# nncarlson/nka

Hardware: AMD Instinct MI355X
Metric: NKA updates/sec + achieved HBM GB/s at n=1e8, m=20 fp64; 1/2/4/8 GPUs (higher is better)
Workload: dtype f64

## Files before the change

### nka_amd/csrc/handles.hpp

```cpp
#pragma once

#include "../../include/nka_hip.h"
#include "../../include/nka_hip_ext.h"
#include "../../include/nka_hip_vec.h"
#include "nka_kernels.hpp"
#include "host_logic.hpp"
#include "rccl_dl.hpp"

#include <hip/hip_runtime.h>

#include <cstdint>
#include <string>
#include <vector>

namespace nka_detail {
int set_error(int code, const std::string &msg);
std::string last_error();
bool &span_check_failed();
int check_device_span(const void *p, int64_t n, const char *what);
void invalidate_span_cache();
void register_allocation(const void *p, size_t bytes, const void *owner);
void unregister_owner(const void *owner);
void unregister_allocation(const void *p);

// ... 41 lines not shown
  bool swap_pending = false;
  int64_t swap_seq = 0;
  const double *last_acc = nullptr;
  std::vector<void *> extra_allocs;
  nka_host::BufferBook book;
  bool captured = false;
  bool solve63_raised = false;
  bool poisoned = false;
  int num_cu = 256;
  int bpc[2] = {0, 0};
  char devname[64] = {0};
  int pa_pipe = -1;
  int pb_pipe = -1;
  int pb_flags = 0;
  int pb_tile = -1;
  int pb_tickets = -1;
  double *chain_pred = nullptr;
  void *chain_summ = nullptr;
  long long chain_cap = 0;
  int chain_many = -1;
  int chain_walk = 0;
  int fail_after_solve = 0;
  int prime_pad = -1;
  bool state_in_global = false;
  bool serial_solve = false;
  int sum_order = NKA_HIP_SUMS_AUTO;
  bool debug = false;
  nka_hip_allreduce_fn allreduce = nullptr;
  void *allreduce_ctx = nullptr;
  ncclComm_t comm = nullptr;
  nka::P2P p2p{};
  void *p2p_mail = nullptr;
  std::vector<void *> p2p_opened;
  void *p2p_dev = nullptr;
  int p2p_ranks = 0;
  bool p2p_fused = false;
  int pa_normed = 0;
  int shard_rank = -1, shard_n = 0;
  bool needs_comm = false;
  nka_hip_host_dot_fn host_dot = nullptr;
  void *host_dot_ctx = nullptr;
  int timing_cap = 0;
  int64_t timing_count = 0;
  int timing_stride = 1;
  int64_t update_seq = 0;
  bool timing_this = false;
// ... 21 lines not shown
```

### nka_amd/csrc/lab.hip

```cpp
#include "handles.hpp"
#include "../../include/nka_hip_diag.h"

#include <algorithm>
#include <string>

using namespace nka;
using namespace nka_detail;

extern "C" {

int nka_hip_get_stamps(nka_hip_t a, double *out16) {
  if (!a || !out16) return fail(NKA_HIP_EINVAL, "null argument");
  HIP_TRY(hipSetDevice(a->device));
  HIP_TRY(hipMemcpyAsync(out16, a->ctl.stamps(), sizeof(double) * kStamps, hipMemcpyDeviceToHost, a->stream));
  HIP_TRY(hipStreamSynchronize(a->stream));
  return 0;
}

int nka_hip_set_grid(nka_hip_t a, int32_t pa, int32_t pb) {
  if (!a) return fail(NKA_HIP_EINVAL, "null handle");
  const int32_t v[2] = {pa, pb};
  for (int i = 0; i < 2; i++) {
    if (v[i] < 0 || v[i] * a->num_cu > kMaxGrid) return fail(NKA_HIP_EINVAL, "blocks per CU out of range");
    a->bpc[i] = v[i];
// ... 73 lines not shown
  } else if (k == "pa_pipe") {
    if (value != -1 && value != 0 && !(value > 200 && value <= 204))
      return fail(NKA_HIP_EINVAL, "pa_pipe: -1 (auto), 0 (every load of a tile in flight), 201..204 (rolling window, 1..4 blocks per CU)");
    a->pa_pipe = value;
  } else if (k == "pb_tile") {
    if (value != -1 && value != 1 && value != 2) return fail(NKA_HIP_EINVAL, "pb_tile: -1 (auto), 1, 2");
    a->pb_tile = value;
  } else if (k == "pb_tickets") {
    if (value != -1 && value != 0 && value != 1 && value != 2 && value != 4 && value != 8)
      return fail(NKA_HIP_EINVAL, "pb_tickets: -1 (auto), 0 (static tile mapping), 1, 2, 4, 8 (ticket counters)");
    a->pb_tickets = value;
  } else if (k == "fail_after_solve") {
    a->fail_after_solve = value != 0;
  } else if (k == "prime_pad") {
    if (value < -1 || value > 1) return fail(NKA_HIP_EINVAL, "prime_pad: -1, 0, 1");
    a->prime_pad = value;
  } else if (k == "chain_many") {
    if (value < -1 || value > 1) return fail(NKA_HIP_EINVAL, "chain_many: -1, 0, 1");
    a->chain_many = value;
  } else if (k == "chain_walk") {
    a->chain_walk = value != 0;
  } else if (k == "serial_solve") {
    a->serial_solve = value != 0;
  } else if (k == "list_word") {
    a->word_off = value == 0;
  } else {
    return fail(NKA_HIP_EINVAL, "unknown tuning key: " + k);
  }
  return 0;
}

int nka_hip_vec_set_tuning(nka_hip_vec_ws_t ws, const char *key, int32_t value) {
  if (!ws || !key) return fail(NKA_HIP_EINVAL, "null argument");
  if (std::string(key) == "tickets") {
    if (value != -1 && value != 0 && value != 1 && value != 2 && value != 4 && value != 8)
      return fail(NKA_HIP_EINVAL, "tickets: -1 (auto), 0 (static tile mapping), 1, 2, 4, 8 (ticket counters)");
    ws->ticket_groups = value;
    return 0;
  }
  return fail(NKA_HIP_EINVAL, std::string("unknown tuning key: ") + key);
}

}
```

### nka_amd/csrc/nka_hip.hip

```cpp
#include "handles.hpp"

#include <dlfcn.h>

#include <algorithm>
#include <atomic>
#include <chrono>
#include <cmath>
#include <cstdio>
#include <cstdlib>
#include <cstring>
#include <map>
#include <mutex>
#include <set>
#include <string>
#include <vector>

using namespace nka;

namespace {
thread_local std::string g_err;
}

namespace nka_detail {
int set_error(int code, const std::string &msg) {
// ... 314 lines not shown
constexpr int kTimingEvents = 4;

int list_bound_now(nka_hip_state *a) {
  if (a->word_off || !a->list_word) return a->list_ub;
  const unsigned long long w = __atomic_load_n(a->list_word, __ATOMIC_ACQUIRE);
  return nka_host::list_bound_from_word(a->list_ub, w, a->seq, a->word_valid_after, a->relaxed_after);
}

constexpr size_t kMaxDynamicLds = 160 * 1024;
constexpr int kMaxMvec = 140;
static_assert(lst_smem_bytes(kMaxMvec) <= kMaxDynamicLds && lst_smem_bytes(kMaxMvec + 1) > kMaxDynamicLds,
              "kMaxMvec out of step with lst_smem_bytes");

int record(nka_hip_state *a, int i) {
  if (i == 0) a->timing_this = a->timing_cap > 0 && (a->update_seq++ % a->timing_stride) == 0;
  if (!a->timing_this) return 0;
  const int slot = (int)(a->timing_count % a->timing_cap);
  HIP_TRY(hipEventRecord(a->ev[(size_t)slot * kTimingEvents + i], a->stream));
  return 0;
}

}

extern "C" {

const char *nka_hip_last_error(void) { return g_err.c_str(); }

void nka_hip_invalidate_pointer_cache(void) { nka_detail::invalidate_span_cache(); }

int nka_hip_create(nka_hip_t *out, int64_t vlen_local, int32_t mvec, double vtol, int32_t flavor,
                   int32_t device, void *stream) {
  if (!out) return fail(NKA_HIP_EINVAL, "nka_hip_create: out is NULL");
  *out = nullptr;
  if (mvec <= 0) return fail(NKA_HIP_EINVAL, "nka_hip_create: mvec must be > 0");
  if (vlen_local < 0) return fail(NKA_HIP_EINVAL, "nka_hip_create: vlen must be >= 0");
  if (!(vtol > 0.0)) return fail(NKA_HIP_EINVAL, "nka_hip_create: vtol must be > 0");
  if (flavor == NKA_HIP_FLAVOR_DEFAULT) {
    flavor = NKA_HIP_FLAVOR_C;
    if (const char *e = getenv("NKA_HIP_FLAVOR")) {
      const std::string v(e);
      if (v == "f08" || v == "F08" || v == "0") flavor = NKA_HIP_FLAVOR_F08;
      else if (v == "f08vec" || v == "F08VEC" || v == "f08_vector" || v == "1") flavor = NKA_HIP_FLAVOR_F08_VECTOR;
      else if (v == "c" || v == "C" || v == "compact" || v == "2") flavor = NKA_HIP_FLAVOR_C;
      else if (!v.empty()) return fail(NKA_HIP_EINVAL, "NKA_HIP_FLAVOR: expected f08, f08vec or c, got '" + v + "'");
    }
  }
// ... 191 lines not shown

static int fetch_tables(nka_hip_t a, std::vector<long long> &pc, Ctl &t) {
  pc.assign((size_t)a->ctl.pc_count(), 0);
  HIP_TRY(hipMemcpyAsync(pc.data(), a->ctl.pc, sizeof(long long) * pc.size(), hipMemcpyDeviceToHost, a->stream));
  HIP_TRY(hipStreamSynchronize(a->stream));
  t = a->ctl;
  t.pc = pc.data();
  return 0;
}
static const double *slot_buffer(nka_hip_t a, const Ctl *tables, bool v, int slot) {
  if (tables) return buffer_at(a, v ? tables->vtab()[slot] : tables->wtab()[slot]);
  return (v ? a->vs.v : a->vs.w) + (size_t)(slot - 1) * a->vs.stride;
}
static __global__ void k_plan_pointers_from_slots(Ctl ctl) {
  if (threadIdx.x != 0 || blockIdx.x != 0) return;
  const int n = ctl.ic[IC_PLAN_NOLDER];
  for (int j = 0; j < n; j++) ctl.plan_w()[j] = ctl.wtab()[ctl.plan_slots()[j]];
  ctl.pc[PC_FIRST_W] = ctl.wtab()[ctl.ic[IC_PLAN_FIRST]];
}

int nka_hip_clone(nka_hip_t src, nka_hip_t *out) {
  if (!src || !out) return fail(NKA_HIP_EINVAL, "nka_hip_clone: null argument");
  *out = nullptr;
  nka_hip_t b = nullptr;
  if (int rc = nka_hip_create(&b, src->n, src->mvec, src->vtol, src->flavor, src->device, (void *)src->stream)) return rc;
  if (b->vs.stride != src->vs.stride || b->ctl.ic_count() != src->ctl.ic_count() || b->ctl.dc_count() != src->ctl.dc_count()) {
    nka_hip_destroy(b);
    return fail(NKA_HIP_ESTATE, "nka_hip_clone: storage geometry differs");
  }
  const size_t slot_bytes = (size_t)src->vs.stride * sizeof(double) * (size_t)(src->mvec + 1);
  hipStream_t s = src->stream;
  hipError_t e = hipSuccess;
  if (!src->swapped) {
    e = hipMemcpyAsync(b->vs.v, src->vs.v, slot_bytes, hipMemcpyDeviceToDevice, s);
    if (e == hipSuccess) e = hipMemcpyAsync(b->vs.w, src->vs.w, slot_bytes, hipMemcpyDeviceToDevice, s);
  } else {
    std::vector<long long> pc;
    Ctl t{};
    if (int rc = fetch_tables(src, pc, t)) {
      nka_hip_destroy(b);
      return rc;
    }
    const size_t nb = sizeof(double) * (size_t)src->n;
    for (int k = 1; k <= src->mvec + 1 && e == hipSuccess && nb > 0; k++) {
      e = hipMemcpyAsync(b->vs.w + (size_t)(k - 1) * b->vs.stride, buffer_at(src, t.wtab()[k]), nb, hipMemcpyDeviceToDevice, s);
      if (e == hipSuccess)
        e = hipMemcpyAsync(b->vs.v + (size_t)(k - 1) * b->vs.stride, buffer_at(src, t.vtab()[k]), nb, hipMemcpyDeviceToDevice, s);
    }
  }
  if (e == hipSuccess) e = hipMemcpyAsync(b->ctl.ic, src->ctl.ic, sizeof(int32_t) * src->ctl.ic_count(), hipMemcpyDeviceToDevice, s);
  if (e == hipSuccess) e = hipMemcpyAsync(b->ctl.dc, src->ctl.dc, sizeof(double) * src->ctl.dc_count(), hipMemcpyDeviceToDevice, s);
  if (e == hipSuccess) {
    hipLaunchKernelGGL(k_plan_pointers_from_slots, dim3(1), dim3(1), 0, s, b->ctl);
    e = hipGetLastError();
  }
  if (e != hipSuccess) {
    nka_hip_destroy(b);
    return fail(NKA_HIP_EHIP, std::string("nka_hip_clone: ") + hipGetErrorString(e));
  }
  b->pending = src->pending;
  b->list_ub = src->list_ub;
  b->bpc[0] = src->bpc[0];
  b->bpc[1] = src->bpc[1];
  b->pa_pipe = src->pa_pipe;
  b->pb_pipe = src->pb_pipe;
  b->pb_tile = src->pb_tile;
  b->pb_tickets = src->pb_tickets;
  b->prime_pad = src->prime_pad;
  b->chain_walk = src->chain_walk;
  b->chain_many = src->chain_many;
  b->chain_pred = nullptr; b->chain_summ = nullptr; b->chain_cap = 0;
  b->serial_solve = src->serial_solve;
  b->sum_order = src->sum_order;
  b->shard_rank = src->shard_rank;
  b->shard_n = src->shard_n;
  b->debug = src->debug;
  if (src->allreduce != rccl_allreduce && src->allreduce != p2p_allreduce) {
    b->allreduce = src->allreduce;
    b->allreduce_ctx = src->allreduce_ctx;
    b->needs_comm = src->needs_comm;
  } else {
    b->needs_comm = true;
  }
  b->host_dot = src->host_dot;
  b->host_dot_ctx = src->host_dot_ctx;
  *out = b;
  return 0;
}

int nka_hip_restart(nka_hip_t a) {
  if (!a) return fail(NKA_HIP_EINVAL, "null handle");
  if (a->poisoned) return fail(NKA_HIP_ESTATE, "restart: an earlier update failed after its scalar step had been enqueued: destroy the handle");
  HIP_TRY(hipSetDevice(a->device));
  hipLaunchKernelGGL(k_restart, dim3(1), dim3(kSolveThreads), a->state_in_global ? 0 : lst_smem_bytes(a->mvec), a->stream,
                     a->ctl, a->state_in_global ? 1 : 0);
  HIP_TRY(hipGetLastError());
  a->pending = false;
  a->list_ub = 0;
  a->word_valid_after = a->seq;
  a->relaxed_after.clear();
  return 0;
}

int nka_hip_relax(nka_hip_t a) {
  if (!a) return fail(NKA_HIP_EINVAL, "null handle");
  if (a->poisoned) return fail(NKA_HIP_ESTATE, "relax: an earlier update failed after its scalar step had been enqueued: destroy the handle");
  HIP_TRY(hipSetDevice(a->device));
  hipLaunchKernelGGL(k_relax, dim3(1), dim3(kSolveThreads), a->state_in_global ? 0 : lst_smem_bytes(a->mvec), a->stream,
                     a->ctl, a->state_in_global ? 1 : 0);
  HIP_TRY(hipGetLastError());
  if (a->pending) {
    a->pending = false;
    a->list_ub = std::max(a->list_ub - 1, 0);
    if (!a->word_off && a->list_word) a->relaxed_after.push_back(a->seq);
    if (a->relaxed_after.size() > 4096) a->relaxed_after.erase(a->relaxed_after.begin(), a->relaxed_after.begin() + 2048);
  }
  return 0;
}

int nka_hip_set_vec_tol(nka_hip_t a, double vtol) {
  if (!a) return fail(NKA_HIP_EINVAL, "null handle");
  if (!(vtol > 0.0)) return fail(NKA_HIP_EINVAL, "set_vec_tol: vtol must be > 0");
  HIP_TRY(hipSetDevice(a->device));
  a->vtol = vtol;
  HIP_TRY(hipMemcpyAsync(a->ctl.dc + DC_VTOL, &a->vtol, sizeof(double), hipMemcpyHostToDevice, a->stream));
  HIP_TRY(hipStreamSynchronize(a->stream));
  return 0;
}

static int enqueue_solve(nka_hip_t a, int mode, long long swap_w = kNoBuffer, long long swap_v = kNoBuffer, bool gather = false) {
  hipStream_t s = a->stream;
  const P2P x = gather ? a->p2p : P2P{};
  if (a->mvec + 1 <= kSolveWaveMax && !a->serial_solve) {
    const size_t sm = solve_wave_smem_bytes(a->mvec);
    const int nl = a->mvec + 1;
    const long long id_stride = (a->swapped || a->captured) ? 0 : (long long)a->vs.stride, id_vbase = buffer_offset(a, a->vs.v);
#define ROWS(NL) \
  hipLaunchKernelGGL((k_solve_rows<NL>), dim3(1), dim3(kSolveThreads), sm, s, a->ctl, mode, swap_w, swap_v, id_stride, id_vbase, x)
    if (nl <= 6) ROWS(6);
    else if (nl <= 11) ROWS(11);
    else if (nl <= 21) ROWS(21);
    else if (nl <= 33) ROWS(33);
    else if (nl <= 48) ROWS(48);
    else {
      if (!a->solve63_raised) {
        const hipError_t raised = hipFuncSetAttribute(reinterpret_cast<const void *>(k_solve_rows<63>),
                                                      hipFuncAttributeMaxDynamicSharedMemorySize,
                                                      (int)solve_wave_smem_bytes(kSolveWaveMax - 1));
        if (raised != hipSuccess) return fail(NKA_HIP_EHIP, std::string("raising the dynamic LDS limit failed: ") + hipGetErrorString(raised));
        a->solve63_raised = true;
      }
      ROWS(63);
    }
#undef ROWS
  } else {
    hipLaunchKernelGGL(k_solve, dim3(1), dim3(kSolveThreads), a->state_in_global ? 0 : lst_smem_bytes(a->mvec), s, a->ctl, mode,
                       a->state_in_global ? 1 : 0, 0, swap_w, swap_v, x);
  }
  HIP_TRY(hipGetLastError());
  return 0;
}

}

void nka_detail::enqueue_pa(nka_hip_t a, const double *f, int vec, int older_ub) {
  const int maxl = (vec == 1) ? 4 : (older_ub > kMaxPerPass ? kMaxPerPass : round_up4(older_ub));
  const int npass = std::max(1, (older_ub + maxl - 1) / maxl);
  int pa_pipe = a->pa_pipe;
  const bool exact = vec == 2 && older_ub >= 1 && older_ub <= kMaxPerPass;
  if (pa_pipe < 0) pa_pipe = exact ? 201 : 0;
  if (vec == 2 && npass == 1 && pa_pipe > 200 && pa_pipe < 210) {
    int w = exact ? older_ub : maxl;
    if (a->prime_pad != 0 && heavy_prime(w)) w++;
    launch_dots_win(w, a, f, std::max(1, pa_pipe - 200));
  } else if (vec == 2 && older_ub > kMaxPerPass && a->pa_pipe != 0) {
    const int np = balanced_passes(older_ub);
    std::vector<int> wd((size_t)np);
    balanced_widths(older_ub, np, wd.data());
    for (int p = 0, base = 0; p < np; p++) {
      launch_dots_win(wd[(size_t)p], a, f, a->pa_pipe > 200 ? a->pa_pipe - 200 : 1, base, p, older_ub);
      base += wd[(size_t)p];
    }
  } else {
    for (int p = 0; p < npass; p++) {
      if (vec == 2) launch_dots_w(maxl, a, f, p, npass);
      else launch_dots_1<4, 1>(a, f, p, npass);
    }
  }
// ... 347 lines not shown
  return r;
}

static SumsResult sums_blocked(nka_hip_t a, const double *f, int vec, int older_ub) {
  SumsResult r;
  if (!(a->pending || older_ub > 0)) return r;
  RoctxRange range("nka:PA dots + all-reduce");
  r.gather = a->allreduce == p2p_allreduce && a->p2p.base != nullptr;
  a->p2p_fused = r.gather;
  enqueue_pa(a, f, vec, older_ub);
  a->p2p_fused = false;
  if (hipError_t e = hipGetLastError(); e != hipSuccess) {
    r.rc = fail(NKA_HIP_EHIP, std::string("accel_update: ") + hipGetErrorString(e));
    return r;
  }
  if (a->allreduce && !r.gather)
    if (int rc = a->allreduce(a->allreduce_ctx, a->ctl.red(), a->ctl.red_count(), a->stream)) r.rc = hook_failed(rc);
  return r;
}

static int update_impl(nka_hip_t a, double *f, long long swap_w, long long swap_v);
static int p2p_status_after_sync(nka_hip_t a);

int nka_hip_accel_update(nka_hip_t a, double *f) { return update_impl(a, f, kNoBuffer, kNoBuffer); }

static int update_impl(nka_hip_t a, double *f, long long swap_w, long long swap_v) {
  if (!a) return fail(NKA_HIP_EINVAL, "null handle");
  if (!f && a->n > 0) return fail(NKA_HIP_EINVAL, "accel_update: f is NULL");
  HIP_TRY(hipSetDevice(a->device));
  if (int rc = nka_detail::check_device_span(f, a->n, "accel_update: f")) return rc;
  if (swap_w == kNoBuffer && f && f == a->last_acc)
    return fail(NKA_HIP_EINVAL, "accel_update: that buffer is the accelerated f lent by the previous out-of-place update (read only: "
                                "it is the stored v of the pending pair); copy it, or go on with nka_hip_accel_update_swap");
  if (a->poisoned)
    return fail(NKA_HIP_ESTATE, "accel_update: an earlier update of this handle failed after its scalar step had been enqueued "
                                "(a HIP error): the lists on the device are ahead of the stored vectors.  Destroy the handle");
  if (a->swapped && f && held_by_library(a, f))
    return fail(NKA_HIP_EINVAL, "accel_update: that buffer is held by the library (a stored vector, or a buffer handed over to "
                                "nka_hip_accel_update_swap earlier)");
  if (a->needs_comm)
    return fail(NKA_HIP_ECOMM, "accel_update: this accelerator is a copy of a sharded one and has no all-reduce yet: call "
                               "nka_hip_comm_init_rank or nka_hip_set_allreduce on it first (nka_hip_clone)");
  const bool chain = a->sum_order == NKA_HIP_SUMS_REFERENCE_ORDER && a->allreduce && !a->host_dot;
  if (chain && (a->shard_n < 1 || a->shard_rank < 0))
    return fail(NKA_HIP_ESTATE, "accel_update: reference-order sums on a sharded accelerator continue the running sums from rank "
                                "to rank: tell the handle where its slice lies in the global vector first (nka_hip_set_shard; "
// ... 3 lines not shown
  if (a->debug && nka_hip_defined(a) != 1)
    return fail(NKA_HIP_ESTATE, "accel_update: the device state fails the defined() invariants");
  hipStream_t s = a->stream;
  const bool aligned = (reinterpret_cast<uintptr_t>(f) % 16) == 0;
  const int vec = aligned ? 2 : 1;
  int mode = (a->flavor == NKA_HIP_FLAVOR_F08_VECTOR) ? kSolveRcp : 0;
  {
    const bool user_hook = a->allreduce && a->allreduce != rccl_allreduce && a->allreduce != p2p_allreduce;
    if (!a->captured || user_hook || a->host_dot) {
      hipStreamCaptureStatus cs = hipStreamCaptureStatusNone;
      if (hipStreamIsCapturing(s, &cs) != hipSuccess) (void)hipGetLastError();
      else if (cs != hipStreamCaptureStatusNone) {
        if (user_hook || a->host_dot)
          return fail(NKA_HIP_EINVAL, "accel_update: cannot be captured into a graph with a caller's all-reduce hook or dot product "
                                      "installed (host callbacks: a replay would not call them); the built-in RCCL hook and the "
                                      "peer-to-peer exchange can be captured");
        a->captured = a->word_off = true;
      }
    }
  }
  if (int rc = record(a, 0)) return rc;
  a->list_ub = list_bound_now(a);
  const int older_ub = a->pending ? std::max(a->list_ub - 1, 0) : a->list_ub;

  SumsResult sums{};
  switch (pick_sums_stage(a)) {
    case SumsStage::HostDot:        sums = sums_host_dot(a, f, mode); break;
    case SumsStage::ReferenceChain: sums = sums_reference_chain(a, f, mode, older_ub); break;
    case SumsStage::ReferenceOrder: sums = sums_reference_order(a, f, mode, older_ub); break;
    case SumsStage::Rounded:        sums = sums_rounded(a, f, vec, mode, older_ub); break;
    case SumsStage::Blocked:        sums = sums_blocked(a, f, vec, older_ub); break;
  }
  if (sums.rc) return sums.rc;
  mode |= sums.mode_bits;
  const bool solved = sums.solved, gather = sums.gather;
  if (int rc = record(a, 1)) return rc;

  RoctxRange range_tail("nka:solve + PB combine");
  if (!solved)
    if (int rc = enqueue_solve(a, mode, swap_w, swap_v, gather)) return rc;
  struct Poison {
    nka_hip_state *a;
    bool armed = true;
    ~Poison() { if (armed) a->poisoned = true; }
  } poison{a};
  if (a->fail_after_solve) {
    a->fail_after_solve = 0;
    return fail(NKA_HIP_EHIP, "accel_update: injected failure behind the scalar step (lab switch fail_after_solve)");
  }
  if (int rc = record(a, 2)) return rc;

  const int comb_ub = a->pending ? std::min(a->list_ub, (int)a->mvec) : a->list_ub;
  a->ctl.seq = (unsigned long long)(a->seq + 1);
  {
    Ctl &c = a->ctl;
    unsigned long long *const hw = c.hw;
    if (a->word_off) c.hw = nullptr;
    a->pb_flags = (swap_w != kNoBuffer ? (kPbNoStoreW | kPbNoStoreF) : 0);
    const int rc = enqueue_pb(a, f, vec, comb_ub);
    a->pb_flags = 0;
    c.hw = hw;
    if (rc) return rc;
  }
  a->seq++;
  if (int rc = record(a, 3)) return rc;

  if (a->timing_this) a->timing_count++;
  a->list_ub = comb_ub + 1;
// ... 123 lines not shown
int nka_hip_num_vec(nka_hip_t a) {
  if (!a) return fail(NKA_HIP_EINVAL, "null handle");
  std::vector<int32_t> ic;
  std::vector<double> dc;
  if (int rc = fetch_state(a, ic, dc)) return rc;
  const int32_t *next = ic.data() + IC_HEADER;
  int n = 0;
  for (int k = ic[IC_FIRST]; k != 0 && n <= a->mvec + 1; k = next[k]) n++;
  return ic[IC_PENDING] ? n - 1 : n;
}

int nka_hip_max_vec(nka_hip_t a) { return a ? a->mvec : fail(NKA_HIP_EINVAL, "null handle"); }
int nka_hip_flavor(nka_hip_t a) { return a ? a->flavor : fail(NKA_HIP_EINVAL, "null handle"); }
int64_t nka_hip_vec_len(nka_hip_t a) { return a ? a->n : (int64_t)fail(NKA_HIP_EINVAL, "null handle"); }
double nka_hip_vec_tol(nka_hip_t a) {
  if (a) return a->vtol;
  fail(NKA_HIP_EINVAL, "null handle");
  return -1.0;
}

int nka_hip_get_state(nka_hip_t a, int32_t *subspace, int32_t *pending, int32_t *first, int32_t *last,
                      int32_t *free_, int32_t *next, int32_t *prev, double *h, double *c) {
  if (!a) return fail(NKA_HIP_EINVAL, "null handle");
  std::vector<int32_t> ic;
  std::vector<double> dc;
  if (int rc = fetch_state(a, ic, dc)) return rc;
  const int m1 = a->mvec + 1;
  if (subspace) *subspace = ic[IC_SUBSPACE];
  if (pending) *pending = ic[IC_PENDING];
  if (first) *first = ic[IC_FIRST];
  if (last) *last = ic[IC_LAST];
  if (free_) *free_ = ic[IC_FREE];
  const int32_t *nx = ic.data() + IC_HEADER, *pv = nx + (m1 + 1);
  const double *hh = dc.data() + DC_HEADER, *cc = hh + (m1 + 1) * (m1 + 1);
  for (int k = 1; k <= m1; k++) {
    if (next) next[k - 1] = nx[k];
    if (prev) prev[k - 1] = pv[k];
    if (c) c[k - 1] = cc[k];
  }
  if (h)
    for (int j = 1; j <= m1; j++)
      for (int i = 1; i <= m1; i++) h[(i - 1) + (size_t)(j - 1) * m1] = hh[i * (m1 + 1) + j];
  return 0;
}

int nka_hip_get_reductions(nka_hip_t a, double *red_out) {
  if (!a || !red_out) return fail(NKA_HIP_EINVAL, "null argument");
  HIP_TRY(hipSetDevice(a->device));
  HIP_TRY(hipMemcpyAsync(red_out, a->ctl.red(), sizeof(double) * a->ctl.red_count(), hipMemcpyDeviceToHost, a->stream));
  HIP_TRY(hipStreamSynchronize(a->stream));
  return 0;
}

int nka_hip_defined(nka_hip_t a) {
  if (!a) return 0;
  std::vector<int32_t> ic;
  std::vector<double> dc;
  if (fetch_state(a, ic, dc)) return 0;
  const int n = a->mvec + 1;
  if (a->mvec < 1 || !a->vs.v || !a->vs.w) return 0;
  if (!(dc[DC_VTOL] > 0.0)) return 0;
  const int32_t *next = ic.data() + IC_HEADER, *prev = next + (n + 1);
  const int first = ic[IC_FIRST], last = ic[IC_LAST], fr = ic[IC_FREE];
  for (int k = 1; k <= n; k++)
    if (next[k] < 0 || next[k] > n) return 0;
  if (first < 0 || first > n || fr < 0 || fr > n) return 0;
  std::vector<char> tag(n + 1, 0);
  if (first == 0) {
    if (last != 0) return 0;
  } else {
    int k = first;
// ... 253 lines not shown
  return 0;
}

int nka_hip_comm_library(char *path, int32_t len) {
  if (!path || len <= 0) return fail(NKA_HIP_EINVAL, "bad buffer");
  if (!rccl().ok()) return fail(NKA_HIP_ECOMM, rccl().err);
  snprintf(path, (size_t)len, "%s", rccl().path.c_str());
  return 0;
}

int nka_hip_allreduce_now(nka_hip_t a, double *buf_dev, int32_t count) {
  if (!a) return fail(NKA_HIP_EINVAL, "null handle");
  if (count < 0) return fail(NKA_HIP_EINVAL, "negative count");
  HIP_TRY(hipSetDevice(a->device));
  if (int rc = nka_detail::check_device_span(buf_dev, count, "allreduce_now: buf")) return rc;
  if (a->allreduce && count > 0)
    if (int rc = a->allreduce(a->allreduce_ctx, buf_dev, count, a->stream))
      return rc < 0 ? rc : fail(NKA_HIP_ECOMM, "allreduce hook failed");
  return 0;
}

int nka_hip_state_digest(nka_hip_t a, uint64_t *digest) {
  if (!a || !digest) return fail(NKA_HIP_EINVAL, "null argument");
  std::vector<int32_t> ic;
  std::vector<double> dc;
  if (int rc = fetch_state(a, ic, dc)) return rc;
  uint64_t h = 1469598103934665603ull;
  auto mix = [&h](const void *p, size_t nbytes) {
    const unsigned char *b = static_cast<const unsigned char *>(p);
    for (size_t i = 0; i < nbytes; i++) {
      h ^= b[i];
      h *= 1099511628211ull;
    }
  };
  mix(ic.data(), ic.size() * sizeof(int32_t));
  mix(dc.data(), dc.size() * sizeof(double));
  *digest = h;
  return 0;
}


int nka_hip_set_timing(nka_hip_t a, int32_t capacity) {
  if (!a) return fail(NKA_HIP_EINVAL, "null handle");
  if (capacity < 0 || capacity > 4096) return fail(NKA_HIP_EINVAL, "timing capacity out of range");
  HIP_TRY(hipSetDevice(a->device));
  HIP_TRY(hipStreamSynchronize(a->stream));
// ... 55 lines not shown
```

### nka_amd/csrc/nka_kernels.hpp

```cpp
#pragma once

#include <hip/hip_runtime.h>
#include <stdint.h>

#if defined(__HIP_DEVICE_COMPILE__) && !defined(__gfx950__)
#error "nka_kernels.hpp is written for gfx950 (CDNA4) only: v_permlane32_swap / v_permlane16_swap reductions, 160 KiB LDS, tile shapes measured on MI355X.  Build with --offload-arch=gfx950."
#endif

namespace nka {

constexpr int kBlock = 256;
constexpr int kWavesPerBlock = kBlock / 64;
constexpr int kMaxGrid = 4096;

enum {
  IC_SUBSPACE = 0,
  IC_PENDING = 1,
  IC_FIRST = 2,
  IC_LAST = 3,
  IC_FREE = 4,
  IC_NEW = 5,
  IC_NCOMB = 6,
  IC_PLAN_PENDING = 7,
  IC_PLAN_FIRST = 8,
  IC_PLAN_NOLDER = 9,
  IC_NRELAX = 10,
  IC_NORMED = 11,
  IC_HEADER = 16
};
enum { DC_VTOL = 0, DC_S = 1, DC_HEADER = 2 };
enum {
  PC_FIRST_W = 0,
  PC_NEW_W = 1,
  PC_NEW_V = 2,
  PC_OLD_W = 3,
  PC_OLD_V = 4,
  PC_HEADER = 8
};

constexpr int kMaxPerPass = 32;

constexpr int kStamps = 16;
#ifdef NKA_SOLVE_STAMPS
#define NKA_STAMP(ctl, i) do { if (threadIdx.x == 0) (ctl).stamps()[i] = (double)__builtin_amdgcn_s_memtime(); } while (0)
#define NKA_STAMP0(ctl, i) do { if (blockIdx.x == 0 && threadIdx.x == 0) (ctl).stamps()[i] = (double)__builtin_amdgcn_s_memtime(); } while (0)
#else
#define NKA_STAMP(ctl, i) do { } while (0)
#define NKA_STAMP0(ctl, i) do { } while (0)
#endif

struct Ctl {
  int32_t *ic;
  double *dc;
  int32_t mvec;
  unsigned long long *hw;
  unsigned long long seq;
  long long *pc;
  __host__ __device__ long long *plan_w() const { return pc + PC_HEADER; }
  __host__ __device__ long long *comb_w() const { return plan_w() + m1p(); }
  __host__ __device__ long long *comb_v() const { return comb_w() + m1p(); }
  __host__ __device__ long long *wtab() const { return comb_v() + m1p(); }
// ... 303 lines not shown
  }
  if (v2) {
    if ((int)blockIdx.x == G - 1)
      for (int64_t i = done + threadIdx.x; i < vs.n; i += kBlock) {
        const double d = w1[i] - f[i];
        acc = fma(d, d, acc);
      }
  } else {
    for (int64_t i = (int64_t)blockIdx.x * kBlock + threadIdx.x; i < vs.n; i += (int64_t)G * kBlock) {
      const double d = w1[i] - f[i];
      acc = fma(d, d, acc);
    }
  }
  const double one[1] = {acc};
  block_reduce_store<1>(one, partials, G);
}
static __global__ __launch_bounds__(64) __attribute__((unused)) void k_norm_fin(Ctl ctl, const double *__restrict__ partials, int G) {
  double r = 0.0;
  for (int b = threadIdx.x; b < G; b += 64) r += partials[b];
  r = wave_sum(r);
  if (threadIdx.x == 0) ctl.red()[0] = ctl.ic[IC_PLAN_PENDING] ? r : 0.0;
}

template <int MAXL, int W>
__global__ __launch_bounds__(kBlock) void k_dots_win(Ctl ctl, Vecs vs, const double *__restrict__ f,
                                                     double *__restrict__ partials, int base, int normed) {
  constexpr int VEC = 2;
  using V = typename VecT<VEC>::type;
  constexpr int NACC = 2 * MAXL + 2;
  static_assert(MAXL % W == 0, "the ring must divide the stored vectors of a tile");
  NKA_STAMP0(ctl, 10);
  const int G = gridDim.x;
  const int pending = ctl.ic[IC_PLAN_PENDING];
  const double s_n = normed ? sqrt(ctl.red()[0]) : 1.0, rs_n = 1.0 / s_n;
  const int nolder = ctl.ic[IC_PLAN_NOLDER] - base;
  const long long *pw = ctl.plan_w() + base;
  const double *w1p = vs.w + ctl.pc[PC_FIRST_W];
  const double *w1 = pending ? w1p : f;
  long long sl[MAXL];
#pragma unroll
  for (int j = 0; j < MAXL; j++) sl[j] = pw[j];
  const double *wk[MAXL];
#pragma unroll
  for (int j = 0; j < MAXL; j++) wk[j] = (j < nolder) ? vs.w + sl[j] : f;
  double acc[NACC];
#pragma unroll
  for (int a = 0; a < NACC; a++) acc[a] = 0.0;

  const int64_t ntile = vs.n / (kBlock * VEC);
#define DEAD_OFF(live, off) (off)
  V fv, w1v, ring[W];
  int64_t t = blockIdx.x;
  if (t < ntile) {
    const int64_t e = t * (kBlock * VEC) + threadIdx.x * VEC;
    fv = ld<VEC>(f + e);
    w1v = ld<VEC>(w1 + e);
#pragma unroll
    for (int j = 0; j < W; j++) ring[j] = ld<VEC>(wk[j] + (DEAD_OFF(j < nolder, e)));
  }
  NKA_STAMP0(ctl, 11);
  for (; t < ntile; t += G) {
    const int64_t e = t * (kBlock * VEC) + threadIdx.x * VEC;
    const int64_t tn = (t + G < ntile) ? t + G : t;
    const int64_t en = tn * (kBlock * VEC) + threadIdx.x * VEC;
    double dq[VEC], fq[VEC];
#pragma unroll
    for (int q = 0; q < VEC; q++) {
      fq[q] = ex(fv, q);
      dq[q] = pa_operand(ex(w1v, q) - fq[q], normed, s_n, rs_n);
      acc[0] = fma(dq[q], dq[q], acc[0]);
      acc[1] = fma(fq[q], dq[q], acc[1]);
    }
    __builtin_amdgcn_sched_barrier(0);
    fv = ld<VEC>(f + en);
    w1v = ld<VEC>(w1 + en);
#pragma unroll
    for (int j = 0; j < MAXL; j++) {
      const V x = ring[j % W];
      __builtin_amdgcn_sched_barrier(0);
      if (j + W < MAXL) ring[j % W] = ld<VEC>(wk[j + W] + (DEAD_OFF(j + W < nolder, e)));
      else ring[j % W] = ld<VEC>(wk[j + W - MAXL] + (DEAD_OFF(j + W - MAXL < nolder, en)));
      __builtin_amdgcn_sched_barrier(0);
#pragma unroll
      for (int q = 0; q < VEC; q++) {
        acc[2 + j] = fma(dq[q], ex(x, q), acc[2 + j]);
        acc[2 + MAXL + j] = fma(fq[q], ex(x, q), acc[2 + MAXL + j]);
      }
    }
  }
  if ((int)blockIdx.x == G - 1) {
    for (int64_t i = ntile * (kBlock * VEC) + threadIdx.x; i < vs.n; i += kBlock) {
      const double fq = f[i];
      const double d = pa_operand(w1[i] - fq, normed, s_n, rs_n);
      acc[0] = fma(d, d, acc[0]);
      acc[1] = fma(fq, d, acc[1]);
#pragma unroll
      for (int j = 0; j < MAXL; j++) {
        const double x = wk[j][i];
        acc[2 + j] = fma(d, x, acc[2 + j]);
        acc[2 + MAXL + j] = fma(fq, x, acc[2 + MAXL + j]);
      }
    }
  }
  NKA_STAMP0(ctl, 12);
  block_reduce_store<NACC>(acc, partials, G);
  NKA_STAMP0(ctl, 13);
#undef DEAD_OFF
}

constexpr int kFinThreads = 64;
template <int MAXL>
__global__ __launch_bounds__(kFinThreads) void k_finalize_dots(Ctl ctl, const double *__restrict__ partials, int G,
                                                               int pass, int ncover, int base, P2P x, int keep0 = 0) {
  const int lane = threadIdx.x;
  const int c = blockIdx.x;
  const bool p2p = x.base != nullptr;
  const unsigned long long xs = p2p ? *x.xseq : 0ull;
  double r = 0.0;
  for (int b = lane; b < G; b += kFinThreads) r += partials[(size_t)c * G + b];
  r = wave_sum(r);
  const int nolder = ctl.ic[IC_PLAN_NOLDER];
  const int pending = ctl.ic[IC_PLAN_PENDING];
  if (pass == 0 && c == 0)
    for (int p = ncover + lane; p < ctl.mvec; p += kFinThreads) {
      if (p2p) {
        for (int q = 0; q < x.n; q++) {
          p2p_send_one(x, q, xs, 2 + p, 0.0);
          p2p_send_one(x, q, xs, 2 + ctl.mvec + p, 0.0);
        }
      } else {
        ctl.red()[2 + p] = 0.0;
        ctl.red()[2 + ctl.mvec + p] = 0.0;
      }
    }
  int dst = -1;
  bool live = false;
  if (c < 2) {
    if (pass == 0 && !(keep0 && c == 0)) { dst = c; live = pending != 0; }
  } else if (c < 2 + MAXL) {
    const int p = base + (c - 2);
    if (p < ctl.mvec) { dst = 2 + p; live = pending && p < nolder; }
  } else {
    const int p = base + (c - 2 - MAXL);
    if (p < ctl.mvec) { dst = 2 + ctl.mvec + p; live = p < nolder; }
  }
  if (dst < 0) return;
  if (p2p) {
    p2p_send_wave(x, xs, dst, live ? readlane_f64(r, 0) : 0.0);
    return;
  }
  if (lane == 0) ctl.red()[dst] = live ? r : 0.0;
}

constexpr int kOrdThreads = 256;
constexpr int kOrdChunkMax = 512;
constexpr int kOrdMaxMvec = 250;
constexpr int kOrdAutoMax = 64;
constexpr int kOrdLdsDoubles = 16000;
constexpr int kOrdLdsPad = 16;
__host__ __device__ inline int ord_chunk(int rows) {
  int c = kOrdLdsDoubles / (rows < 1 ? 1 : rows) - 1;
  return c > kOrdChunkMax ? kOrdChunkMax : (c < 8 ? 8 : c);
}
__host__ __device__ inline size_t ord_lds_bytes(int rows) {
  return sizeof(double) * ((size_t)rows * (ord_chunk(rows) + 1) + kOrdLdsPad);
}
__device__ __forceinline__ double ord_sum(double a, const double *x, const double *y, int len) {
#pragma clang fp contract(off)
  double xb[8], yb[8];
#pragma unroll
  for (int u = 0; u < 8; u++) { xb[u] = x[u]; yb[u] = y[u]; }
  for (int i0 = 0; i0 < len; i0 += 8) {
    double xn[8], yn[8];
#pragma unroll
// ... 1229 lines not shown
  long long *wt = ctl.wtab(), *vt = ctl.vtab();
  if (swap_w != kNoBuffer) { ctl.pc[PC_OLD_W] = wt[slot]; wt[slot] = swap_w; }
  if (swap_v != kNoBuffer) { ctl.pc[PC_OLD_V] = vt[slot]; vt[slot] = swap_v; }
  ctl.pc[PC_NEW_W] = wt[slot];
  ctl.pc[PC_NEW_V] = vt[slot];
}

static __global__ __launch_bounds__(kSolveThreads) __attribute__((unused)) void k_restart(Ctl ctl, int in_global) {
  extern __shared__ __attribute__((aligned(16))) unsigned char smem[];
  Lst L;
  lst_load(L, ctl, smem, in_global);
  if (threadIdx.x == 0) lst_restart(L);
  lst_store(L, ctl, in_global);
}

static __global__ __launch_bounds__(kSolveThreads) __attribute__((unused)) void k_relax(Ctl ctl, int in_global) {
  extern __shared__ __attribute__((aligned(16))) unsigned char smem[];
  Lst L;
  lst_load(L, ctl, smem, in_global);
  if (threadIdx.x == 0) lst_relax(L);
  lst_store(L, ctl, in_global);
}

enum { kSolveRcp = 1, kSolvePrenorm = 2 };
__device__ __forceinline__ double solve_nrm(double x, double s, double rs, int mode) {
  return (mode & kSolvePrenorm) ? x : ((mode & kSolveRcp) ? rs * x : x / s);
}

static __global__ __launch_bounds__(kSolveThreads) __attribute__((unused)) void k_solve(Ctl ctl, int mode, int in_global,
                                                                                       int phase, long long swap_w,
                                                                                       long long swap_v, P2P x) {
  extern __shared__ __attribute__((aligned(16))) unsigned char smem[];
  if (x.base != nullptr) p2p_gather_block(x, ctl.red(), ctl.red_count());
  Lst L;
  lst_load(L, ctl, smem, in_global);
  if (threadIdx.x == 0) {
    const double *red = ctl.red();
    const int32_t *ps = ctl.plan_slots();
    const int nolder = ctl.ic[IC_PLAN_NOLDER];
    const int entry_first = L.first;
    bool normed = (phase == 2) ? ctl.ic[IC_NORMED] != 0 : false;
    double s = (phase == 2) ? ctl.dc[DC_S] : 0.0;
    if (phase != 2) {
      if (L.pending) {
        s = sqrt(red[0]);
        ctl.dc[DC_S] = s;
        if (s == 0.0) {
// ... 31 lines not shown
      ctl.ic[IC_NCOMB] = ncomb;
      ctl.ic[IC_NEW] = slot;
      assign_new_buffers(ctl, slot, swap_w, swap_v);
      lst_prepend(L, slot);
    }
  }
  lst_store(L, ctl, in_global);
}

constexpr int kSolveWaveMax = 63;

__host__ __device__ inline size_t solve_wave_smem_bytes(int mvec) {
  const int nl = mvec + 1;
  size_t b = (lst_smem_bytes(mvec) + 15) / 16 * 16;
  b += (size_t)((nl + 1) * (nl + 1) + 3 * nl + (2 + 2 * mvec)) * sizeof(double);
  b += (size_t)(3 * nl + 1) * sizeof(int32_t);
  b = (b + 7) / 8 * 8;
  b += (size_t)(2 * (nl + 1)) * sizeof(long long);
  return b;
}

template <int NLMAX>
__global__ __launch_bounds__(kSolveThreads) void k_solve_rows(Ctl ctl, int mode, long long swap_w, long long swap_v,
                                                              long long id_stride, long long id_vbase, P2P x) {
  extern __shared__ __attribute__((aligned(16))) unsigned char smem[];
  const int lane = threadIdx.x;
  if (x.base != nullptr) p2p_gather_block(x, ctl.red(), ctl.red_count());
  const int m1 = ctl.m1(), NL = m1, LDA = NL + 1, M = ctl.mvec, nh = (m1 + 1) * (m1 + 1);
  Lst L;
  L.m1 = m1;
  L.mvec = M;
  L.h = reinterpret_cast<double *>(smem);
  L.c = L.h + nh;
  L.next = reinterpret_cast<int32_t *>(L.c + (m1 + 1));
  L.prev = L.next + (m1 + 1);
  double *A = reinterpret_cast<double *>(smem + (lst_smem_bytes(ctl.mvec) + 15) / 16 * 16);
  double *bb = A + (NL + 1) * LDA + 2 * NL;
  double *redL = bb + NL;
  int32_t *ord = reinterpret_cast<int32_t *>(redL + (2 + 2 * M));
  int32_t *psL = ord + 2 * NL;
  long long *wtL = reinterpret_cast<long long *>((reinterpret_cast<uintptr_t>(psL + NL + 1) + 7) / 8 * 8);
  long long *vtL = wtL + (m1 + 1);
  NKA_STAMP(ctl, 0);
  const int nolder = ctl.ic[IC_PLAN_NOLDER];
  {
    constexpr int kHB = 8;
    static_assert(kSolveWaveMax + 1 <= kSolveThreads, "lists: one load a lane");
    const double *gh = ctl.h(), *gred = ctl.red();
// ... 20 lines not shown
#pragma unroll
    for (int k = 0; k < kHB; k++)
      if (lane + kSolveThreads * k < nh) L.h[lane + kSolveThreads * k] = hreg[k];
#pragma unroll
    for (int k = 0; k < 2; k++)
      if (lane + kSolveThreads * k < 2 + 2 * M) redL[lane + kSolveThreads * k] = rreg[k];
    if (lane < m1 + 1) {
      L.c[lane] = creg;
      L.next[lane] = nreg;
      L.prev[lane] = preg;
      wtL[lane] = wtreg;
      vtL[lane] = vtreg;
    }
    if (lane < nolder) psL[lane] = psreg;
    for (int i = lane + kSolveThreads * kHB; i < nh; i += kSolveThreads) L.h[i] = gh[i];
  }
  L.subspace = ctl.ic[IC_SUBSPACE];
  L.pending = ctl.ic[IC_PENDING];
  L.first = ctl.ic[IC_FIRST];
  L.last = ctl.ic[IC_LAST];
  L.free_ = ctl.ic[IC_FREE];
  L.vtol = ctl.dc[DC_VTOL];
  const int entry_pending = L.pending;
  __syncthreads();
  NKA_STAMP(ctl, 1);
  const double vtol2 = L.vtol * L.vtol;

  const int entry_first = L.first;
  int normed = 0;
  double s = 0.0;
  if (L.pending) {
    s = sqrt(redL[0]);
    if (s == 0.0) lst_relax(L);
  }
  if (L.pending) normed = 1;
  {
    const double rs = 1.0 / s;
    for (int p = lane; p < nolder; p += kSolveThreads) {
      if (normed) L.H(L.first, psL[p]) = solve_nrm(redL[2 + p], s, rs, mode);
      L.c[psL[p]] = redL[2 + M + p];
    }
    if (normed && lane == 0) L.c[entry_first] = solve_nrm(redL[1], s, rs, mode);
  }
  __syncthreads();
  const int nl = normed ? 1 + nolder : 0;
  const int myord = normed ? (lane == 0 ? entry_first : (lane <= nolder ? psL[lane - 1] : 0)) : 0;
// ... 66 lines not shown
    if (lane < nl) yr = A[nl * LDA + lane];
    forward_done = true;
    for (uint64_t dm = ~alive & listmask & ~1ull; dm != 0; dm &= dm - 1) {
      const int p = __builtin_ctzll(dm);
      const int k = __builtin_amdgcn_readlane(myord, p);
      if (p == capdrop) {
        L.next[L.last] = L.free_;
        L.free_ = k;
        L.last = L.prev[k];
        L.next[L.last] = 0;
      } else {
        const int pv = L.prev[k], nx = L.next[k];
        L.next[pv] = nx;
        if (nx == 0) L.last = pv; else L.prev[nx] = pv;
        L.next[k] = L.free_;
        L.free_ = k;
      }
    }
    L.subspace = 1;
    L.pending = 0;
    __syncthreads();
  }

  NKA_STAMP(ctl, 5);
  const int slot = L.free_;
  L.free_ = L.next[slot];
  const long long new_w = swap_w != kNoBuffer ? swap_w : wtL[slot], new_v = swap_v != kNoBuffer ? swap_v : vtL[slot];
  if (lane == 0) {
    if (swap_w != kNoBuffer) ctl.pc[PC_OLD_W] = wtL[slot];
    if (swap_v != kNoBuffer) ctl.pc[PC_OLD_V] = vtL[slot];
    ctl.pc[PC_NEW_W] = new_w;
    ctl.pc[PC_NEW_V] = new_v;
    ctl.pc[PC_FIRST_W] = new_w;
    if (swap_w != kNoBuffer) ctl.wtab()[slot] = swap_w;
    if (swap_v != kNoBuffer) ctl.vtab()[slot] = swap_v;
  }
  if (forward_done) {
    NKA_STAMP(ctl, 6);
    double t[NLMAX];
#pragma unroll
    for (int i = 0; i < NLMAX; i++) t[i] = A[(i < nl ? i : nl) * LDA + (lane < nl ? lane : nl)];
#pragma unroll
    for (int i = NLMAX - 1; i >= 0; i--) {
      if (i < nl && ((alive >> i) & 1)) {
        const double ci = readlane_f64(yr, i) / readlane_f64(Ldr, i);
        if (lane == i) yr = ci;
        if (lane < i && ((alive >> lane) & 1)) yr = yr - t[i] * ci;
      }
    }
    NKA_STAMP(ctl, 7);
    nk = __builtin_popcountll(alive & listmask);
// ... 74 lines not shown
```

Before: 134.7.

## Speculatively skip dot products against the vector about to be dropped

```diff
diff --git a/nka_amd/csrc/handles.hpp b/nka_amd/csrc/handles.hpp
--- a/nka_amd/csrc/handles.hpp
+++ b/nka_amd/csrc/handles.hpp
@@ -87,6 +87,11 @@
   int chain_walk = 0;
   int fail_after_solve = 0;
   int prime_pad = -1;
+  int pa_skip = -1;
+  bool pa_spec = false;
+  const double *skip_f = nullptr;
+  bool skip_used = false;
+  double *skip_spare = nullptr;
   bool state_in_global = false;
   bool serial_solve = false;
   int sum_order = NKA_HIP_SUMS_AUTO;
diff --git a/nka_amd/csrc/lab.hip b/nka_amd/csrc/lab.hip
--- a/nka_amd/csrc/lab.hip
+++ b/nka_amd/csrc/lab.hip
@@ -119,6 +119,9 @@
     a->chain_walk = value != 0;
   } else if (k == "serial_solve") {
     a->serial_solve = value != 0;
+  } else if (k == "pa_skip_dropped") {
+    if (value < -1 || value > 1) return fail(NKA_HIP_EINVAL, "pa_skip_dropped: -1, 0, 1");
+    a->pa_skip = value;
   } else if (k == "list_word") {
     a->word_off = value == 0;
   } else {
diff --git a/nka_amd/csrc/nka_hip.hip b/nka_amd/csrc/nka_hip.hip
--- a/nka_amd/csrc/nka_hip.hip
+++ b/nka_amd/csrc/nka_hip.hip
@@ -360,6 +360,24 @@
 
 }
 
+static int skip_grid(const nka_hip_state *a) {
+  const int64_t ntile = a->n / (kBlock * 2);
+  return (int)std::max<int64_t>(1, std::min<int64_t>(std::min<int64_t>(a->num_cu, std::max<int64_t>(ntile, 1)), kMaxGrid));
+}
+static void complete_skip_at(nka_hip_t a, int rec_at) {
+  const int g = skip_grid(a);
+  hipLaunchKernelGGL((k_dots_win<1, 1, 2>), dim3(g), dim3(kBlock), 0, a->stream, a->ctl, a->vs, (const double *)nullptr, a->partials,
+                     rec_at, 0);
+  hipLaunchKernelGGL(k_skip_patch, dim3(1), dim3(2 * kFinThreads), 0, a->stream, a->ctl, a->partials, g, rec_at);
+}
+static int complete_skip(nka_hip_t a) {
+  if (!a->skip_used) return 0;
+  HIP_TRY(hipSetDevice(a->device));
+  complete_skip_at(a, PC_SKIP_CUR);
+  HIP_TRY(hipGetLastError());
+  return 0;
+}
+
 extern "C" {
 
 const char *nka_hip_last_error(void) { return g_err.c_str(); }
@@ -597,6 +615,7 @@
 int nka_hip_clone(nka_hip_t src, nka_hip_t *out) {
   if (!src || !out) return fail(NKA_HIP_EINVAL, "nka_hip_clone: null argument");
   *out = nullptr;
+  if (int rc = complete_skip(src)) return rc;
   nka_hip_t b = nullptr;
   if (int rc = nka_hip_create(&b, src->n, src->mvec, src->vtol, src->flavor, src->device, (void *)src->stream)) return rc;
   if (b->vs.stride != src->vs.stride || b->ctl.ic_count() != src->ctl.ic_count() || b->ctl.dc_count() != src->ctl.dc_count()) {
@@ -642,6 +661,7 @@
   b->pb_tile = src->pb_tile;
   b->pb_tickets = src->pb_tickets;
   b->prime_pad = src->prime_pad;
+  b->pa_skip = src->pa_skip;
   b->chain_walk = src->chain_walk;
   b->chain_many = src->chain_many;
   b->chain_pred = nullptr; b->chain_summ = nullptr; b->chain_cap = 0;
@@ -667,6 +687,7 @@
   if (!a) return fail(NKA_HIP_EINVAL, "null handle");
   if (a->poisoned) return fail(NKA_HIP_ESTATE, "restart: an earlier update failed after its scalar step had been enqueued: destroy the handle");
   HIP_TRY(hipSetDevice(a->device));
+  if (int rc = complete_skip(a)) return rc;
   hipLaunchKernelGGL(k_restart, dim3(1), dim3(kSolveThreads), a->state_in_global ? 0 : lst_smem_bytes(a->mvec), a->stream,
                      a->ctl, a->state_in_global ? 1 : 0);
   HIP_TRY(hipGetLastError());
@@ -681,6 +702,7 @@
   if (!a) return fail(NKA_HIP_EINVAL, "null handle");
   if (a->poisoned) return fail(NKA_HIP_ESTATE, "relax: an earlier update failed after its scalar step had been enqueued: destroy the handle");
   HIP_TRY(hipSetDevice(a->device));
+  if (int rc = complete_skip(a)) return rc;
   hipLaunchKernelGGL(k_relax, dim3(1), dim3(kSolveThreads), a->state_in_global ? 0 : lst_smem_bytes(a->mvec), a->stream,
                      a->ctl, a->state_in_global ? 1 : 0);
   HIP_TRY(hipGetLastError());
@@ -703,7 +725,8 @@
   return 0;
 }
 
-static int enqueue_solve(nka_hip_t a, int mode, long long swap_w = kNoBuffer, long long swap_v = kNoBuffer, bool gather = false) {
+static int enqueue_solve(nka_hip_t a, int mode, long long swap_w = kNoBuffer, long long swap_v = kNoBuffer, bool gather = false,
+                         int gate = 0) {
   hipStream_t s = a->stream;
   const P2P x = gather ? a->p2p : P2P{};
   if (a->mvec + 1 <= kSolveWaveMax && !a->serial_solve) {
@@ -711,7 +734,7 @@
     const int nl = a->mvec + 1;
     const long long id_stride = (a->swapped || a->captured) ? 0 : (long long)a->vs.stride, id_vbase = buffer_offset(a, a->vs.v);
 #define ROWS(NL) \
-  hipLaunchKernelGGL((k_solve_rows<NL>), dim3(1), dim3(kSolveThreads), sm, s, a->ctl, mode, swap_w, swap_v, id_stride, id_vbase, x)
+  hipLaunchKernelGGL((k_solve_rows<NL>), dim3(1), dim3(kSolveThreads), sm, s, a->ctl, mode, swap_w, swap_v, id_stride, id_vbase, x, gate)
     if (nl <= 6) ROWS(6);
     else if (nl <= 11) ROWS(11);
     else if (nl <= 21) ROWS(21);
@@ -739,6 +762,10 @@
 }
 
 void nka_detail::enqueue_pa(nka_hip_t a, const double *f, int vec, int older_ub) {
+  if (a->pa_spec) {
+    launch_dots_win(a->mvec - 1, a, f, 1);
+    return;
+  }
   const int maxl = (vec == 1) ? 4 : (older_ub > kMaxPerPass ? kMaxPerPass : round_up4(older_ub));
   const int npass = std::max(1, (older_ub + maxl - 1) / maxl);
   int pa_pipe = a->pa_pipe;
@@ -1132,6 +1159,46 @@
 static int update_impl(nka_hip_t a, double *f, long long swap_w, long long swap_v);
 static int p2p_status_after_sync(nka_hip_t a);
 
+static bool skip_eligible(const nka_hip_state *a, int vec, int older_ub) {
+  return a->pa_skip != 0 && pick_sums_stage(a) == SumsStage::Rounded && !a->allreduce && !a->host_dot && vec == 2 && a->pending &&
+         older_ub == a->mvec && a->mvec >= 2 && a->mvec <= kMaxPerPass && !heavy_prime(a->mvec - 1) &&
+         (a->pa_pipe < 0 || a->pa_pipe == 201) && !a->serial_solve && a->n > 0;
+}
+
+static bool skip_spare_ready(nka_hip_t a) {
+  if (a->skip_spare) return true;
+  if (a->captured) return false;
+  void *q = nullptr;
+  if (hipMalloc(&q, sizeof(double) * (size_t)a->vs.stride) != hipSuccess) {
+    (void)hipGetLastError();
+    return false;
+  }
+  const long long off = buffer_offset(a, static_cast<double *>(q));
+  if (hipMemcpy(a->ctl.pc + PC_SPARE_W, &off, sizeof off, hipMemcpyHostToDevice) != hipSuccess) {
+    (void)hipGetLastError();
+    hipFree(q);
+    return false;
+  }
+  a->extra_allocs.push_back(q);
+  a->book.taken.insert(static_cast<const double *>(q));
+  a->skip_spare = static_cast<double *>(q);
+  a->swapped = true;
+  return true;
+}
+
+static int enqueue_skip_fallback(nka_hip_t a, int mode) {
+  const int g = skip_grid(a);
+  const int base = a->mvec - 1;
+  hipLaunchKernelGGL((k_dots_win<1, 1, 1>), dim3(g), dim3(kBlock), 0, a->stream, a->ctl, a->vs, a->skip_f, a->partials, base,
+                     (mode & kSolveRcp) ? 3 : 1);
+  hipLaunchKernelGGL((k_finalize_dots<1>), dim3(4), dim3(kFinThreads), 0, a->stream, a->ctl, a->partials, g, 1, 1, base, P2P{}, 1, 1);
+  HIP_TRY(hipGetLastError());
+  if (int rc = enqueue_solve(a, mode & ~kSolveSpec, kNoBuffer, kNoBuffer, false, 1)) return rc;
+  complete_skip_at(a, PC_SKIP_PREV);
+  HIP_TRY(hipGetLastError());
+  return 0;
+}
+
 int nka_hip_accel_update(nka_hip_t a, double *f) { return update_impl(a, f, kNoBuffer, kNoBuffer); }
 
 static int update_impl(nka_hip_t a, double *f, long long swap_w, long long swap_v) {
@@ -1181,8 +1248,14 @@
   if (int rc = record(a, 0)) return rc;
   a->list_ub = list_bound_now(a);
   const int older_ub = a->pending ? std::max(a->list_ub - 1, 0) : a->list_ub;
+  const bool spec = swap_w == kNoBuffer && skip_eligible(a, vec, older_ub) && skip_spare_ready(a);
+  if (!spec)
+    if (int rc = complete_skip(a)) return rc;
+  a->skip_used = a->skip_used || spec;
 
   SumsResult sums{};
+  a->pa_spec = spec;
+  a->skip_f = f;
   switch (pick_sums_stage(a)) {
     case SumsStage::HostDot:        sums = sums_host_dot(a, f, mode); break;
     case SumsStage::ReferenceChain: sums = sums_reference_chain(a, f, mode, older_ub); break;
@@ -1190,6 +1263,7 @@
     case SumsStage::Rounded:        sums = sums_rounded(a, f, vec, mode, older_ub); break;
     case SumsStage::Blocked:        sums = sums_blocked(a, f, vec, older_ub); break;
   }
+  a->pa_spec = false;
   if (sums.rc) return sums.rc;
   mode |= sums.mode_bits;
   const bool solved = sums.solved, gather = sums.gather;
@@ -1197,12 +1271,14 @@
 
   RoctxRange range_tail("nka:solve + PB combine");
   if (!solved)
-    if (int rc = enqueue_solve(a, mode, swap_w, swap_v, gather)) return rc;
+    if (int rc = enqueue_solve(a, mode | (spec ? kSolveSpec : 0), swap_w, swap_v, gather)) return rc;
   struct Poison {
     nka_hip_state *a;
     bool armed = true;
     ~Poison() { if (armed) a->poisoned = true; }
   } poison{a};
+  if (spec)
+    if (int rc = enqueue_skip_fallback(a, mode)) return rc;
   if (a->fail_after_solve) {
     a->fail_after_solve = 0;
     return fail(NKA_HIP_EHIP, "accel_update: injected failure behind the scalar step (lab switch fail_after_solve)");
@@ -1372,6 +1448,7 @@
 int nka_hip_get_state(nka_hip_t a, int32_t *subspace, int32_t *pending, int32_t *first, int32_t *last,
                       int32_t *free_, int32_t *next, int32_t *prev, double *h, double *c) {
   if (!a) return fail(NKA_HIP_EINVAL, "null handle");
+  if (int rc = complete_skip(a)) return rc;
   std::vector<int32_t> ic;
   std::vector<double> dc;
   if (int rc = fetch_state(a, ic, dc)) return rc;
@@ -1397,6 +1474,7 @@
 int nka_hip_get_reductions(nka_hip_t a, double *red_out) {
   if (!a || !red_out) return fail(NKA_HIP_EINVAL, "null argument");
   HIP_TRY(hipSetDevice(a->device));
+  if (int rc = complete_skip(a)) return rc;
   HIP_TRY(hipMemcpyAsync(red_out, a->ctl.red(), sizeof(double) * a->ctl.red_count(), hipMemcpyDeviceToHost, a->stream));
   HIP_TRY(hipStreamSynchronize(a->stream));
   return 0;
@@ -1696,6 +1774,7 @@
 
 int nka_hip_state_digest(nka_hip_t a, uint64_t *digest) {
   if (!a || !digest) return fail(NKA_HIP_EINVAL, "null argument");
+  if (int rc = complete_skip(a)) return rc;
   std::vector<int32_t> ic;
   std::vector<double> dc;
   if (int rc = fetch_state(a, ic, dc)) return rc;
diff --git a/nka_amd/csrc/nka_kernels.hpp b/nka_amd/csrc/nka_kernels.hpp
--- a/nka_amd/csrc/nka_kernels.hpp
+++ b/nka_amd/csrc/nka_kernels.hpp
@@ -35,8 +35,13 @@
   PC_NEW_V = 2,
   PC_OLD_W = 3,
   PC_OLD_V = 4,
-  PC_HEADER = 8
+  PC_SPARE_W = 5,
+  PC_FALLBACK = 6,
+  PC_SKIP_CUR = 7,
+  PC_SKIP_PREV = PC_SKIP_CUR + 6,
+  PC_HEADER = 24
 };
+enum { SK_LIVE = 0, SK_W1 = 1, SK_F = 2, SK_WD = 3, SK_H = 4, SK_C = 5 };
 
 constexpr int kMaxPerPass = 32;
 
@@ -386,20 +391,27 @@
   if (threadIdx.x == 0) ctl.red()[0] = ctl.ic[IC_PLAN_PENDING] ? r : 0.0;
 }
 
-template <int MAXL, int W>
+template <int MAXL, int W, int SRC = 0>
 __global__ __launch_bounds__(kBlock) void k_dots_win(Ctl ctl, Vecs vs, const double *__restrict__ f,
                                                      double *__restrict__ partials, int base, int normed) {
   constexpr int VEC = 2;
   using V = typename VecT<VEC>::type;
   constexpr int NACC = 2 * MAXL + 2;
   static_assert(MAXL % W == 0, "the ring must divide the stored vectors of a tile");
+  static_assert(SRC == 0 || MAXL == 1, "the fallback and completion columns are one entry wide");
+  const long long *rec = ctl.pc + base;
+  if (SRC == 1 && ctl.pc[PC_FALLBACK] == 0) return;
+  if (SRC == 2) {
+    if (rec[SK_LIVE] == 0) return;
+    f = vs.w + rec[SK_F];
+  }
   NKA_STAMP0(ctl, 10);
   const int G = gridDim.x;
-  const int pending = ctl.ic[IC_PLAN_PENDING];
+  const int pending = SRC == 2 ? 1 : ctl.ic[IC_PLAN_PENDING];
   const double s_n = normed ? sqrt(ctl.red()[0]) : 1.0, rs_n = 1.0 / s_n;
-  const int nolder = ctl.ic[IC_PLAN_NOLDER] - base;
-  const long long *pw = ctl.plan_w() + base;
-  const double *w1p = vs.w + ctl.pc[PC_FIRST_W];
+  const int nolder = SRC == 2 ? 1 : ctl.ic[IC_PLAN_NOLDER] - base;
+  const long long *pw = SRC == 2 ? rec + SK_WD : ctl.plan_w() + base;
+  const double *w1p = vs.w + (SRC == 2 ? rec[SK_W1] : ctl.pc[PC_FIRST_W]);
   const double *w1 = pending ? w1p : f;
   long long sl[MAXL];
 #pragma unroll
@@ -431,7 +443,7 @@
 #pragma unroll
     for (int q = 0; q < VEC; q++) {
       fq[q] = ex(fv, q);
-      dq[q] = pa_operand(ex(w1v, q) - fq[q], normed, s_n, rs_n);
+      dq[q] = SRC == 2 ? ex(w1v, q) : pa_operand(ex(w1v, q) - fq[q], normed, s_n, rs_n);
       acc[0] = fma(dq[q], dq[q], acc[0]);
       acc[1] = fma(fq[q], dq[q], acc[1]);
     }
@@ -455,7 +467,7 @@
   if ((int)blockIdx.x == G - 1) {
     for (int64_t i = ntile * (kBlock * VEC) + threadIdx.x; i < vs.n; i += kBlock) {
       const double fq = f[i];
-      const double d = pa_operand(w1[i] - fq, normed, s_n, rs_n);
+      const double d = SRC == 2 ? w1[i] : pa_operand(w1[i] - fq, normed, s_n, rs_n);
       acc[0] = fma(d, d, acc[0]);
       acc[1] = fma(fq, d, acc[1]);
 #pragma unroll
@@ -473,16 +485,21 @@
 }
 
 constexpr int kFinThreads = 64;
+__device__ __forceinline__ double fin_column(const double *__restrict__ partials, int c, int G, int lane) {
+  double r = 0.0;
+  for (int b = lane; b < G; b += kFinThreads) r += partials[(size_t)c * G + b];
+  return wave_sum(r);
+}
 template <int MAXL>
 __global__ __launch_bounds__(kFinThreads) void k_finalize_dots(Ctl ctl, const double *__restrict__ partials, int G,
-                                                               int pass, int ncover, int base, P2P x, int keep0 = 0) {
+                                                               int pass, int ncover, int base, P2P x, int keep0 = 0,
+                                                               int gate = 0) {
+  if (gate && ctl.pc[PC_FALLBACK] == 0) return;
   const int lane = threadIdx.x;
   const int c = blockIdx.x;
   const bool p2p = x.base != nullptr;
   const unsigned long long xs = p2p ? *x.xseq : 0ull;
-  double r = 0.0;
-  for (int b = lane; b < G; b += kFinThreads) r += partials[(size_t)c * G + b];
-  r = wave_sum(r);
+  const double r = fin_column(partials, c, G, lane);
   const int nolder = ctl.ic[IC_PLAN_NOLDER];
   const int pending = ctl.ic[IC_PLAN_PENDING];
   if (pass == 0 && c == 0)
@@ -514,6 +531,22 @@
     return;
   }
   if (lane == 0) ctl.red()[dst] = live ? r : 0.0;
+}
+
+static __global__ __launch_bounds__(2 * kFinThreads) __attribute__((unused)) void k_skip_patch(Ctl ctl, const double *__restrict__ partials,
+                                                                                               int G, int rec_at) {
+  long long *rec = ctl.pc + rec_at;
+  if (rec[SK_LIVE] == 0) return;
+  const int lane = threadIdx.x & (kFinThreads - 1), col = threadIdx.x / kFinThreads;
+  const double r = fin_column(partials, 2 + col, G, lane);
+  if (lane == 0) {
+    const int M = ctl.mvec;
+    if (rec_at == PC_SKIP_CUR) ctl.red()[2 + col * M + (M - 1)] = r;
+    const long long at = rec[col == 0 ? SK_H : SK_C];
+    if (at >= 0) (col == 0 ? ctl.h() : ctl.c())[at] = r;
+  }
+  __syncthreads();
+  if (threadIdx.x == 0) rec[SK_LIVE] = 0;
 }
 
 constexpr int kOrdThreads = 256;
@@ -1789,7 +1822,7 @@
   lst_store(L, ctl, in_global);
 }
 
-enum { kSolveRcp = 1, kSolvePrenorm = 2 };
+enum { kSolveRcp = 1, kSolvePrenorm = 2, kSolveSpec = 4 };
 __device__ __forceinline__ double solve_nrm(double x, double s, double rs, int mode) {
   return (mode & kSolvePrenorm) ? x : ((mode & kSolveRcp) ? rs * x : x / s);
 }
@@ -1867,8 +1900,9 @@
 
 template <int NLMAX>
 __global__ __launch_bounds__(kSolveThreads) void k_solve_rows(Ctl ctl, int mode, long long swap_w, long long swap_v,
-                                                              long long id_stride, long long id_vbase, P2P x) {
+                                                              long long id_stride, long long id_vbase, P2P x, int gate) {
   extern __shared__ __attribute__((aligned(16))) unsigned char smem[];
+  if (gate && ctl.pc[PC_FALLBACK] == 0) return;
   const int lane = threadIdx.x;
   if (x.base != nullptr) p2p_gather_block(x, ctl.red(), ctl.red_count());
   const int m1 = ctl.m1(), NL = m1, LDA = NL + 1, M = ctl.mvec, nh = (m1 + 1) * (m1 + 1);
@@ -1935,6 +1969,8 @@
   L.free_ = ctl.ic[IC_FREE];
   L.vtol = ctl.dc[DC_VTOL];
   const int entry_pending = L.pending;
+  const long long prev_live = ctl.pc[PC_SKIP_CUR + SK_LIVE];
+  const long long spare_w = (mode & kSolveSpec) ? ctl.pc[PC_SPARE_W] : kNoBuffer;
   __syncthreads();
   NKA_STAMP(ctl, 1);
   const double vtol2 = L.vtol * L.vtol;
@@ -2047,11 +2083,41 @@
     __syncthreads();
   }
 
+  const bool skipped = (mode & kSolveSpec) && nolder == M;
+  if (skipped && !(normed && capdrop == M)) {
+    if (lane == 0) ctl.pc[PC_FALLBACK] = 1;
+    return;
+  }
+
   NKA_STAMP(ctl, 5);
   const int slot = L.free_;
   L.free_ = L.next[slot];
-  const long long new_w = swap_w != kNoBuffer ? swap_w : wtL[slot], new_v = swap_v != kNoBuffer ? swap_v : vtL[slot];
+  const long long new_w = swap_w != kNoBuffer ? swap_w : skipped ? spare_w : wtL[slot];
+  const long long new_v = swap_v != kNoBuffer ? swap_v : vtL[slot];
   if (lane == 0) {
+    if (prev_live) {
+      long long *cur = ctl.pc + PC_SKIP_CUR, *prv = ctl.pc + PC_SKIP_PREV;
+      const bool h_stale = !(normed && ((alive >> 1) & 1)), c_stale = !normed;
+      prv[SK_W1] = cur[SK_W1];
+      prv[SK_F] = cur[SK_F];
+      prv[SK_WD] = cur[SK_WD];
+      prv[SK_H] = h_stale ? cur[SK_H] : -1;
+      prv[SK_C] = c_stale ? cur[SK_C] : -1;
+      prv[SK_LIVE] = (h_stale || c_stale) ? 1 : 0;
+      cur[SK_LIVE] = 0;
+    }
+    if (skipped) {
+      long long *cur = ctl.pc + PC_SKIP_CUR;
+      cur[SK_W1] = wtL[entry_first];
+      cur[SK_F] = new_w;
+      cur[SK_WD] = wtL[slot];
+      cur[SK_H] = (long long)entry_first * (m1 + 1) + slot;
+      cur[SK_C] = slot;
+      cur[SK_LIVE] = 1;
+      ctl.pc[PC_SPARE_W] = wtL[slot];
+      ctl.wtab()[slot] = new_w;
+    }
+    if (gate) ctl.pc[PC_FALLBACK] = 0;
     if (swap_w != kNoBuffer) ctl.pc[PC_OLD_W] = wtL[slot];
     if (swap_v != kNoBuffer) ctl.pc[PC_OLD_V] = vtL[slot];
     ctl.pc[PC_NEW_W] = new_w;
```

New measurement: 135.2 (median of 6 runs). No clear change (+0.4%).
